# stevenmiller888/mlx-audio

Measured on AMD Instinct MI355X. Metric: audio-sec/sec (xRT), Kokoro-82M batch=32 fixed 128-phoneme utterances per GPU, higher is better.
Workload: dtype bf16; 1 GPU; Kokoro-82M bf16, batch=32/GPU fixed 128-phoneme utterances (T=130, F=650, 390000 samples = 16.25 s each), utterance-sharded over 1 GPU(s); global_batch=32, parallelism=utterance-shard x1, 2 batches in flight per GPU

## Files before the change

mlx-audio_amd/csrc/kk_conv_mfma4.hip:

```cpp
#include <stdlib.h>

#include "kk_common.h"
#include "kk_kernels.h"
#include "kk_conv_mfma_shared.h"

#define TR_NOW() 0ull
#define TR_ADD(slot, v) do { } while (0)
namespace {
typedef __bf16 bf16x2 __attribute__((ext_vector_type(2)));

typedef __bf16 bf16x8 __attribute__((ext_vector_type(8)));
typedef float f32x4 __attribute__((ext_vector_type(4)));

constexpr int BN = 128, CK = 64;
constexpr int XLD = 80;
constexpr int MAX_HALO = 50;
constexpr int CLD = BN;

constexpr int PS_BYTES = 2 * 3 * CK * 4;

template <int BM>
struct Geo {
  static constexpr int XROWS = BM + MAX_HALO;
  static constexpr int XS_BYTES = XROWS * XLD * 2;
  static constexpr int MAIN_BYTES = XS_BYTES + PS_BYTES;
  static constexpr int RPP = BM / 2;
  static constexpr int EPI_BYTES = RPP * CLD * 4;
  static constexpr int LDS_BYTES = MAIN_BYTES > EPI_BYTES ? MAIN_BYTES : EPI_BYTES;
  static constexpr int XREG = (XROWS * 8 + 255) / 256;
};


union U16 {
  uint4 u;
  bf16_t h[8];
};
union U32x8 {
  uint4 u[2];
  float f[8];
};

template <typename TO, int WM, int NRM>
__global__ __launch_bounds__(256, 2) __attribute__((amdgpu_waves_per_eu(2, 2))) void conv_mfma4_kernel(KKMfmaArgs a) {
  constexpr int BM = 2 * WM, MI16 = WM / 16;
  constexpr bool ACC16 = true;
  using G = Geo<BM>;
  constexpr int XREG = G::XREG;
  extern __shared__ __attribute__((aligned(16))) unsigned char smem[];
  bf16_t* Xs = (bf16_t*)smem;
  float* Ps = (float*)(smem + G::XS_BYTES);
  float* Cs = (float*)smem;

  const int tid = threadIdx.x, lane = tid & 63, wave = tid >> 6;
  const int wr = wave >> 1, wc = wave & 1;
  const int nphase = a.mode == KK_CONVT ? a.stride : 1;
  int bx, by, bz;
  {
    const int gx = gridDim.x, gy = gridDim.y, total = gx * gy * gridDim.z;
    int lid = blockIdx.x + gx * (blockIdx.y + gy * blockIdx.z);
    const int per = total / 8, rem = total - per * 8;
    const int xcd = lid & 7, idx = lid >> 3;
    lid = xcd * per + (xcd < rem ? xcd : rem) + idx;
    by = lid % gy;
    const int t = lid / gy;
    bx = t % gx;
    bz = t / gx;
  }
  const int b = bz / nphase, phase = bz - b * nphase;
  const int q0 = bx * BM, n0 = by * BN;
  const int Lin = kk_len(a.lin, b), Lout = kk_len(a.lout, b);

  int ntaps, off0, dstep, widx0, wstep;
  if (a.mode == KK_CONV) {
    ntaps = a.Kw; off0 = -a.pad; dstep = a.dil; widx0 = 0; wstep = 1;
  } else {
    const int k0 = (phase + a.pad) % a.stride;
    ntaps = (a.Kw - k0 + a.stride - 1) / a.stride;
    off0 = (phase + a.pad - k0) / a.stride; dstep = -1; widx0 = k0; wstep = a.stride;
  }
  const int min_off = dstep >= 0 ? off0 : off0 + (ntaps - 1) * dstep;
  const int halo = (ntaps - 1) * (dstep >= 0 ? dstep : -dstep);
  const int xrows = BM + halo;

  const int op_first = a.mode == KK_CONV ? q0 : phase + a.stride * q0;
  const bool tile_live = op_first < Lout;

  const unsigned long long tr0 = TR_NOW();
  unsigned long long tr_sx = 0, tr_sw = 0;
  (void)tr0; (void)tr_sx; (void)tr_sw;
  f32x4 acc[MI16][4];
#pragma unroll
  for (int i = 0; i < MI16; ++i)
#pragma unroll
    for (int j = 0; j < 4; ++j) acc[i][j] = f32x4{0.f, 0.f, 0.f, 0.f};

  if (tile_live) {
    const bf16_t* xb = a.x + (long long)b * a.xbs;
    const int nchunk = a.CinP / CK;
    const int nit = nchunk * ntaps;
    const int lin_hi = Lin > 0 ? Lin - 1 : 0;
    const int cin_real = a.Cin > 0 ? a.Cin : a.CinP;

#define KK_STG(name) name
#define KK_STG_XS Xs
#include "kk_conv_mfma_stage.h"
    uint4 q00, q01, q02, q03, q10, q11, q12, q13;
    const int nb = by;
    auto frag_ptr = [&](int it) __attribute__((always_inline)) -> const uint4* {
      const int chunk = it / ntaps, tap = it - chunk * ntaps;
      const long long blk = ((long long)(widx0 + tap * wstep) * (a.CoutP / BN) + nb) * nchunk + chunk;
      return (const uint4*)a.wf + blk * 1024 + (wc * 2) * 4 * 64 + lane;
    };
    load_x(0);
    {
      const uint4* fp = frag_ptr(0);
      q00 = fp[0 * 64]; q01 = fp[1 * 64]; q02 = fp[2 * 64]; q03 = fp[3 * 64];
      q10 = fp[4 * 64]; q11 = fp[5 * 64]; q12 = fp[6 * 64]; q13 = fp[7 * 64];
      asm volatile("" ::: "memory");
    }
    store_p(0);
    __syncthreads();
    store_x(0);
    __syncthreads();

    const int arow = wr * WM + (lane & 15);
    const int kofs = 8 * (lane >> 4);

    for (int it = 0; it < nit; ++it) {
      const int chunk = it / ntaps, tap = it - chunk * ntaps;
      const bool last_tap = tap == ntaps - 1;
      if (tap == 0 && chunk + 1 < nchunk) load_x(chunk + 1);
      const uint4* fn = frag_ptr(it + 1 < nit ? it + 1 : it);

      const int shift = (off0 + tap * dstep) - min_off;
      const bf16_t* xa = Xs + (arow + shift) * XLD + kofs;
      KK_MFMA_ITER(q00, q01, q02, q03, q10, q11, q12, q13)
      asm volatile("" ::: "memory");
      if (it + 1 < nit) {
        if (tap == 0 && chunk + 1 < nchunk) store_p(chunk + 1);
        if (last_tap) {
          __syncthreads();
          store_x(chunk + 1);
          __syncthreads();
        }
      }
    }
    __syncthreads();
  }

#include "kk_conv_mfma_epilogue.h"
}

template <int XR>
struct GeoWK {
  static constexpr int SROWS = XR == 7 ? 224 : 192 + MAX_HALO;
  static constexpr int SLAB = SROWS * XLD;
  static constexpr int XS_BYTES = 2 * SLAB * 2;
  static constexpr int MAIN_BYTES = XS_BYTES + PS_BYTES;
  static constexpr int RPP = 96;
  static constexpr int EPI_BYTES = RPP * CLD * 4;
  static constexpr int LDS_BYTES = MAIN_BYTES > EPI_BYTES ? MAIN_BYTES : EPI_BYTES;
};

template <int NRM, int XR>
__global__ __launch_bounds__(256, 2) __attribute__((amdgpu_waves_per_eu(2, 2))) void conv_mfma4_wholek_kernel(KKMfmaArgs a) {
  using TO = bf16_t;
  constexpr int WM = 96, BM = 2 * WM, MI16 = WM / 16, XREG = XR;
  constexpr bool ACC16 = true;
  using G = GeoWK<XR>;
  extern __shared__ __attribute__((aligned(16))) unsigned char smem[];
  bf16_t* Xs = (bf16_t*)smem;
  float* Ps = (float*)(smem + G::XS_BYTES);
  float* Cs = (float*)smem;

  const int tid = threadIdx.x, lane = tid & 63, wave = tid >> 6;
  const int wr = wave >> 1, wc = wave & 1;
  constexpr int nphase = 1, phase = 0;
  int bx, by, b;
  {
    const int gx = gridDim.x, gy = gridDim.y, total = gx * gy * gridDim.z;
    int lid = blockIdx.x + gx * (blockIdx.y + gy * blockIdx.z);
    const int per = total / 8, rem = total - per * 8;
    const int xcd = lid & 7, idx = lid >> 3;
    lid = xcd * per + (xcd < rem ? xcd : rem) + idx;
    by = lid % gy;
    const int t = lid / gy;
    bx = t % gx;
    b = t / gx;
  }
  const int q0 = bx * BM, n0 = by * BN;
  const int Lin = kk_len(a.lin, b), Lout = kk_len(a.lout, b);
  const int ntaps = a.Kw, off0 = -a.pad, dstep = a.dil, min_off = off0;
  const int xrows = BM + (ntaps - 1) * dstep;
  const bool tile_live = q0 < Lout;

  const unsigned long long tr0 = TR_NOW();
  (void)tr0;
  f32x4 acc[MI16][4];
#pragma unroll
  for (int i = 0; i < MI16; ++i)
#pragma unroll
    for (int j = 0; j < 4; ++j) acc[i][j] = f32x4{0.f, 0.f, 0.f, 0.f};

  if (tile_live) {
    const bf16_t* xb = a.x + (long long)b * a.xbs;
    const int nit = 2 * ntaps;
    const int lin_hi = Lin > 0 ? Lin - 1 : 0;
    const int cin_real = a.Cin > 0 ? a.Cin : a.CinP;

#define KK_STG(name) name##_s0
#define KK_STG_XS Xs
#include "kk_conv_mfma_stage.h"
#define KK_STG(name) name##_s1
#define KK_STG_XS (Xs + G::SLAB)
#include "kk_conv_mfma_stage.h"
    uint4 q00, q01, q02, q03, q10, q11, q12, q13;
    auto frag_ptr = [&](int it) __attribute__((always_inline)) -> const uint4* {
      const int chunk = it >= ntaps ? 1 : 0, tap = it - chunk * ntaps;
      const long long blk = ((long long)tap * (a.CoutP / BN) + by) * 2 + chunk;
      return (const uint4*)a.wf + blk * 1024 + (wc * 2) * 4 * 64 + lane;
    };
    load_x_s0(0);
    load_x_s1(1);
    {
      const uint4* fp = frag_ptr(0);
      q00 = fp[0 * 64]; q01 = fp[1 * 64]; q02 = fp[2 * 64]; q03 = fp[3 * 64];
      q10 = fp[4 * 64]; q11 = fp[5 * 64]; q12 = fp[6 * 64]; q13 = fp[7 * 64];
      asm volatile("" ::: "memory");
    }
    store_p_s0(0);
    store_p_s1(1);
    __syncthreads();
    store_x_s0(0);
    store_x_s1(1);
    __syncthreads();

    const int arow = wr * WM + (lane & 15);
    const int kofs = 8 * (lane >> 4);
    for (int it = 0; it + 1 < nit; ++it) {
      const int chunk = it >= ntaps ? 1 : 0, tap = it - chunk * ntaps;
      const uint4* fn = frag_ptr(it + 1);
      const bf16_t* xa = Xs + chunk * G::SLAB + (arow + tap * dstep) * XLD + kofs;
      KK_MFMA_ITER(q00, q01, q02, q03, q10, q11, q12, q13)
      asm volatile("" ::: "memory");
    }
    {
      const bf16_t* xa = Xs + G::SLAB + (arow + (ntaps - 1) * dstep) * XLD + kofs;
      KK_MFMA_ITER_LAST(q00, q01, q02, q03, q10, q11, q12, q13)
      asm volatile("" ::: "memory");
    }
    __syncthreads();
  }

#include "kk_conv_mfma_epilogue.h"
}

template <int NRM, int XR>
int launch_wholek(const KKMfmaArgs& a, int B, hipStream_t st) {
  using G = GeoWK<XR>;
  static KKDevOnce attr_once;
  if (attr_once.first()) {
    (void)hipFuncSetAttribute((const void*)conv_mfma4_wholek_kernel<NRM, XR>, hipFuncAttributeMaxDynamicSharedMemorySize, G::LDS_BYTES);
    attr_once.done();
  }
  dim3 grid(kk_cdiv(a.Q, 192), a.CoutP / BN, B);
  hipLaunchKernelGGL((conv_mfma4_wholek_kernel<NRM, XR>), grid, dim3(256), G::LDS_BYTES, st, a);
  KK_CHECK_LAUNCH();
  return 0;
}

template <typename TO, int WM, int NRM>
int launch_one(const KKMfmaArgs& a, int B, hipStream_t st) {
  using G = Geo<2 * WM>;
  static KKDevOnce attr_once;
  if (attr_once.first()) {
    (void)hipFuncSetAttribute((const void*)conv_mfma4_kernel<TO, WM, NRM>, hipFuncAttributeMaxDynamicSharedMemorySize, G::LDS_BYTES);
    attr_once.done();
  }
  const int nphase = a.mode == KK_CONVT ? a.stride : 1;
  dim3 grid(kk_cdiv(a.Q, 2 * WM), a.CoutP / BN, B * nphase);
  hipLaunchKernelGGL((conv_mfma4_kernel<TO, WM, NRM>), grid, dim3(256), G::LDS_BYTES, st, a);
  KK_CHECK_LAUNCH();
  return 0;
}

__global__ __launch_bounds__(256) void pack_w_frag_kernel(const bf16_t* w, bf16_t* wf, int Kw, int CoutP, int CinP) {
  const long long n = (long long)Kw * CoutP * CinP;
  for (long long e = (long long)blockIdx.x * 256 + threadIdx.x; e < n; e += (long long)gridDim.x * 256) {
    const int k = (int)(e % CinP);
    const long long r = e / CinP;
    const int cout = (int)(r % CoutP), tap = (int)(r / CoutP);
    wf[KK_MFMA4_PACK_INDEX(tap, cout, k, CoutP, CinP)] = w[e];
  }
}
}

int kk_launch_pack_w_frag(const void* w, void* wf, int Kw, int CoutP, int CinP, hipStream_t st) {
  if (CinP % CK != 0 || CoutP % BN != 0) return kk_fail("pack_w_frag: CinP must be a multiple of 64 and CoutP of 128");
  hipLaunchKernelGGL(pack_w_frag_kernel, dim3(1024), dim3(256), 0, st, (const bf16_t*)w, (bf16_t*)wf, Kw, CoutP, CinP);
  KK_CHECK_LAUNCH();
  return 0;
}

bool kk_mfma4_wholek_eligible(const KKMfmaArgs& a) {
  return a.mode == KK_CONV && a.stride == 1 && a.CinP == 2 * CK && a.dil >= 1 && (a.Kw - 1) * a.dil <= MAX_HALO;
}

int kk_launch_conv_mfma4(const KKMfmaArgs& a, int B, int out_dtype, hipStream_t st) {
  if (a.Q <= 0 || B <= 0) return 0;
  if (!a.wf) return kk_fail("conv_mfma4: fragment-order weights missing");
  const int nrm = a.nrm_a == nullptr ? 0 : (a.nrm_act == KK_ACT_SNAKE ? 1 : 2);
  if (nrm == 1 && a.nrm_C % 4 != 0) return kk_fail("conv_mfma: the fused Snake input needs a channel count that is a multiple of 4");
  KKMfmaArgs g = a;
  if (nrm == 2 && a.nrm_act != KK_ACT_LRELU) g.nrm_slope = 1.0f;
  if (out_dtype != KK_BF16) return kk_fail("conv_mfma4: bf16 output only");
  if (kk_mfma4_wholek_eligible(g) && !g.slabwise) {
    const bool x7 = (g.Kw - 1) * g.dil <= 32;
    if (nrm == 1) return x7 ? launch_wholek<1, 7>(g, B, st) : launch_wholek<1, 8>(g, B, st);
    if (nrm == 2) return x7 ? launch_wholek<2, 7>(g, B, st) : launch_wholek<2, 8>(g, B, st);
    return x7 ? launch_wholek<0, 7>(g, B, st) : launch_wholek<0, 8>(g, B, st);
  }
  if (nrm == 1) return launch_one<bf16_t, 96, 1>(g, B, st);
  if (nrm == 2) return launch_one<bf16_t, 96, 2>(g, B, st);
  return launch_one<bf16_t, 96, 0>(g, B, st);
}
```

mlx-audio_amd/csrc/kk_model.hip:

```cpp
#include <math.h>
#include <stdio.h>
#include <string.h>

#include <algorithm>
#include <functional>
#include <map>
#include <string>
#include <vector>

#include "../../include/kokoro_hip.h"
#include "kk_common.h"
#include "kk_kernels.h"
#include "kk_host.h"

static thread_local std::string g_err;
static const void* g_op_wfrag = nullptr;
static float g_op_post_slope = 0.f;
static int g_op_variant = 4;

int kk_fail(const char* msg) {
  g_err = msg ? msg : "unknown error";
  return -1;
}
extern "C" const char* kk_last_error(void) { return g_err.c_str(); }
// ... 527 lines not shown
  m->emb_ln_w = P.a.vec("bert.embeddings.LayerNorm.weight", E);
  m->emb_ln_b = P.a.vec("bert.embeddings.LayerNorm.bias", E);
  m->map_in = P.linear("bert.encoder.embedding_hidden_mapping_in", hs, E, true);
  const std::string lp = "bert.encoder.albert_layer_groups.0.albert_layers.0.";
  {
    std::vector<float> w((size_t)3 * hs * hs), b((size_t)3 * hs);
    const char* nm[3] = {"query", "key", "value"};
    for (int i = 0; i < 3; ++i) {
      std::vector<float> wi, bi;
      if (P.read(lp + "attention." + nm[i] + ".weight", (size_t)hs * hs, wi) && P.read(lp + "attention." + nm[i] + ".bias", hs, bi)) {
        memcpy(&w[(size_t)i * hs * hs], wi.data(), wi.size() * 4);
        memcpy(&b[(size_t)i * hs], bi.data(), bi.size() * 4);
      }
    }
    m->qkv = P.pack_oki(w, 3 * hs, 1, hs, &b);
    P.pack_fp8(m->qkv, w, 3 * hs, hs);
  }
  m->att_dense = P.linear(lp + "attention.dense", hs, hs, true);
  m->att_ln_w = P.a.vec(lp + "attention.LayerNorm.weight", hs);
  m->att_ln_b = P.a.vec(lp + "attention.LayerNorm.bias", hs);
  m->full_ln_w = P.a.vec(lp + "full_layer_layer_norm.weight", hs);
  m->full_ln_b = P.a.vec(lp + "full_layer_layer_norm.bias", hs);
  m->ffn = P.linear(lp + "ffn", c.plbert_intermediate, hs, true);
  m->ffn_out = P.linear(lp + "ffn_output", hs, c.plbert_intermediate, true);
  m->bert_encoder = P.linear("bert_encoder", H, hs, true);
  for (int i = 0; i < c.n_layer; ++i) {
    m->dur_lstms.push_back(P.lstm("predictor.text_encoder.lstms." + std::to_string(2 * i), H + S, H / 2));
    m->dur_adaln.push_back(SP.add("predictor.text_encoder.lstms." + std::to_string(2 * i + 1), H));
  }
  m->pred_lstm = P.lstm("predictor.lstm", H + S, H / 2);
  m->shared_lstm = P.lstm("predictor.shared", H + S, H / 2);
  {
    std::vector<float> wd, wt((size_t)c.max_dur * H);
    if (P.read("predictor.duration_proj.linear_layer.weight", (size_t)c.max_dur * H, wd)) {
      for (int o = 0; o < c.max_dur; ++o)
        for (int i = 0; i < H; ++i) wt[(size_t)i * c.max_dur + o] = wd[(size_t)o * H + i];
      m->dur_W = P.put(wt);
    }
  }
  m->dur_b = P.a.vec("predictor.duration_proj.linear_layer.bias", c.max_dur);
  for (int which = 0; which < 2; ++which) {
    const std::string nm = which == 0 ? "predictor.F0" : "predictor.N";
    ResBlk1d* blk = which == 0 ? m->f0blk : m->nblk;
    blk[0] = build_resblk1d(P, SP, nm + ".0", H, H, false);
    blk[1] = build_resblk1d(P, SP, nm + ".1", H, H / 2, true);
    blk[2] = build_resblk1d(P, SP, nm + ".2", H / 2, H / 2, false);
    (which == 0 ? m->f0_proj : m->n_proj) = P.conv_plain(nm + "_proj", 1, 1, H / 2);
  }
  m->te_emb = P.a.vec("text_encoder.embedding.weight", (size_t)c.n_token * H);
  for (int i = 0; i < c.n_layer; ++i) {
    const std::string is = std::to_string(i);
    m->te_cnn.push_back(P.convw("text_encoder.cnn." + is + ".0", H, c.text_encoder_kernel_size, H, true));
    m->te_ln_w.push_back(P.a.vec("text_encoder.cnn." + is + ".1.weight", H));
    m->te_ln_b.push_back(P.a.vec("text_encoder.cnn." + is + ".1.bias", H));
  }
  m->text_lstm = P.lstm("text_encoder.lstm", H, H / 2);
  m->enc = build_resblk1d(P, SD, "decoder.encode", H + 2, DH, false);
  for (int i = 0; i < 3; ++i) m->dec[i] = build_resblk1d(P, SD, "decoder.decode." + std::to_string(i), DH + 2 + 64, DH, false);
  m->dec[3] = build_resblk1d(P, SD, "decoder.decode.3", DH + 2 + 64, H, true);
  m->f0_conv = P.convw("decoder.F0_conv", 1, 3, 1, true);
  m->n_conv = P.convw("decoder.N_conv", 1, 3, 1, true);
  m->asr_res = P.convw("decoder.asr_res.0", 64, 1, H, true);
  const std::string g = "decoder.generator.";
  {
    std::vector<float> lw, lb;
    if (P.read(g + "m_source.l_linear.weight", 9, lw) && P.read(g + "m_source.l_linear.bias", 1, lb)) {
      m->lin_w = P.put(lw);
      m->lin_b = lb[0];
    }
  }
  const int C0 = c.upsample_initial_channel, nk = c.n_resblock_kernels;
  const int d135[3] = {1, 3, 5};
  for (int i = 0; i < c.n_upsamples; ++i) {
    const int cin = C0 >> i, cout = C0 >> (i + 1);
    const std::string is = std::to_string(i);
    m->ups[i] = P.convw_t(g + "ups." + is, cin, c.upsample_kernel_sizes[i], cout);
    if (i + 1 < c.n_upsamples) {
      int sf0 = 1;
      for (int j = i + 1; j < c.n_upsamples; ++j) sf0 *= c.upsample_rates[j];
      m->noise_conv[i] = P.conv_plain(g + "noise_convs." + is, cout, sf0 * 2, c.gen_istft_n_fft + 2);
      m->noise_conv_rows[i] = P.strided_rows(g + "noise_convs." + is, cout, sf0 * 2, c.gen_istft_n_fft + 2, sf0, (sf0 + 1) / 2, 64, &m->noise_rows_pad[i]);
      m->noise_res[i] = build_resblock1(P, SD, g + "noise_res." + is, cout, 7, d135);
    } else {
      m->noise_conv[i] = P.conv_plain(g + "noise_convs." + is, cout, 1, c.gen_istft_n_fft + 2);
      m->noise_res[i] = build_resblock1(P, SD, g + "noise_res." + is, cout, 11, d135);
    }
    for (int j = 0; j < nk; ++j)
      m->resblocks.push_back(
          build_resblock1(P, SD, g + "resblocks." + std::to_string(i * nk + j), cout, c.resblock_kernel_sizes[j], c.resblock_dilations[j]));
  }
  m->conv_post = P.convw(g + "conv_post", c.gen_istft_n_fft + 2, 7, C0 >> c.n_upsamples, true);
  if (P.ok() && m->adt == KK_BF16 && m->conv_post.mfma &&
      kk_head_eligible(m->conv_post.Cin, m->conv_post.Cout, m->conv_post.Kw, c.gen_istft_n_fft, c.gen_istft_hop_size)) {
    const ConvW& cp = m->conv_post;
    m->head_wf_off = P.a.alloc((kk_head_pack_elems() + 1) / 2);
    const uint16_t* src = (const uint16_t*)&P.a.pack[cp.wb_off];
    uint16_t* dst = (uint16_t*)&P.a.pack[m->head_wf_off];
    for (int t = 0; t < cp.Kw; ++t)
      for (int o = 0; o < cp.Cout; ++o)
        for (int i = 0; i < cp.Cin; ++i) dst[kk_head_pack_index(t, o, i)] = src[((size_t)t * cp.CoutP + o) * cp.CinP + i];
  }
  if (P.ok()) {
    SP.build(P, m->sp_wT, m->sp_b, m->Np);
    SD.build(P, m->sd_wT, m->sd_b, m->Nd);
  }
  if (!P.ok()) return kk_failf("kk_finalize: %s", P.a.err.c_str());

  KK_TRY(m->arena.upload((hipStream_t)stream, "kk_finalize"));
  ArenaVec* vecs[] = {&m->emb_word, &m->emb_pos, &m->emb_type, &m->emb_ln_w, &m->emb_ln_b, &m->att_ln_w, &m->att_ln_b, &m->full_ln_w,
                  &m->full_ln_b, &m->dur_W, &m->dur_b, &m->te_emb, &m->lin_w, &m->sp_wT, &m->sp_b, &m->sd_wT, &m->sd_b};
  for (ArenaVec* v : vecs) resolve(m, *v);
  ConvW* convs[] = {&m->map_in, &m->qkv, &m->att_dense, &m->ffn, &m->ffn_out, &m->bert_encoder, &m->f0_proj, &m->n_proj,
                    &m->f0_conv, &m->n_conv, &m->asr_res, &m->conv_post};
  for (ConvW* cw : convs) resolve(m, *cw);
  m->head_wf = m->head_wf_off ? (const bf16_t*)(m->arena.dev + m->head_wf_off) : nullptr;
  for (auto& l : m->dur_lstms) resolve(m, l);
  resolve(m, m->pred_lstm); resolve(m, m->shared_lstm); resolve(m, m->text_lstm);
  for (int i = 0; i < 3; ++i) { resolve(m, m->f0blk[i]); resolve(m, m->nblk[i]); }
  for (auto& cw : m->te_cnn) resolve(m, cw);
  for (auto& v : m->te_ln_w) resolve(m, v);
  for (auto& v : m->te_ln_b) resolve(m, v);
  resolve(m, m->enc);
  for (int i = 0; i < 4; ++i) resolve(m, m->dec[i]);
  for (int i = 0; i < c.n_upsamples; ++i) { resolve(m, m->noise_conv[i]); resolve(m, m->noise_conv_rows[i]); resolve(m, m->ups[i]); resolve(m, m->noise_res[i]); }
  for (auto& r : m->resblocks) resolve(m, r);
  m->finalized = true;
  return 0;
}

namespace {

struct Buf {
  void* p = nullptr;
  int ld = 0;
  long long bs = 0;
  int rows = 0;
  int dtype = KK_F32;
  Buf slice(int coff) const {
    Buf r = *this;
    r.p = p ? (char*)p + (size_t)coff * (dtype == KK_F32 ? 4 : 2) : nullptr;
    return r;
  }
  Buf row_offset(int r0) const {
    Buf r = *this;
    r.p = p ? (char*)p + (size_t)r0 * ld * (dtype == KK_F32 ? 4 : 2) : nullptr;
    r.rows = rows - r0;
    return r;
  }
};

struct ConvOpt {
  int mode = KK_CONV, stride = 1, pad = 0, dil = 1, in_shift = 0;
  float in_slope = 1.f;
  int act = KK_ACT_NONE;
  float act_slope = 0.f;
  float scale = 1.f;
  int accumulate = 0;
  const Buf* res = nullptr;
  const float* nrm_a = nullptr;
  const float* nrm_b = nullptr;
  int nrm_act = KK_ACT_NONE;
  float nrm_slope = 0.f;
  const float* nrm_alpha = nullptr;
  int nrm_C = 0;
  bool want_stats = false;
  bool pad_out_ok = false;
  double alg_taps_cin = 0;
  float post_slope = 1.f;
};

struct Ctx : Workspace {
  kk_model* m;
  kk_context* cx = nullptr;
  hipStream_t st;
  hipStream_t main_st = nullptr;
  bool side_on() const { return !dry && !cx->no_side && cx->side_stream && st != nullptr; }
  int fork_point(int k) {
    if (!side_on()) return 0;
    return hipEventRecord(cx->side_fork[k], st) == hipSuccess ? 0 : kk_fail("kk_forward: hipEventRecord failed");
  }
  int begin_side(int k) {
    if (!side_on()) return 0;
    if (hipStreamWaitEvent(cx->side_stream, cx->side_fork[k], 0) != hipSuccess) return kk_fail("kk_forward: hipStreamWaitEvent failed");
    main_st = st;
    st = cx->side_stream;
    return 0;
  }
  int end_side(int k) {
    if (!side_on() || !main_st) return 0;
    const hipError_t e = hipEventRecord(cx->side_join[k], st);
    st = main_st;
    main_st = nullptr;
    return e == hipSuccess ? 0 : kk_fail("kk_forward: hipEventRecord failed");
  }
  int join_side(int k) {
    if (!side_on()) return 0;
    return hipStreamWaitEvent(st, cx->side_join[k], 0) == hipSuccess ? 0 : kk_fail("kk_forward: hipStreamWaitEvent failed");
  }
  int B;
  int adt;

  Buf act(int rows, int ld, int dtype = -1) {
    Buf b;
    b.dtype = dtype < 0 ? adt : dtype;
    b.ld = ld;
    b.rows = rows;
    b.bs = (long long)rows * ld;
    b.p = raw((size_t)B * rows * ld * (b.dtype == KK_F32 ? 4 : 2));
    return b;
  }
  float* f32(size_t n) { return (float*)raw(n * 4); }
  int* i32(size_t n) { return (int*)raw(n * 4); }

  void prof_start() {
    if (dry || !cx->prof_on) return;
    const size_t i = cx->prof_rec.size();
    if (2 * i + 1 >= cx->prof_ev.size()) return;
    (void)hipEventRecord(cx->prof_ev[2 * i], st);
  }
  void prof_stop(int cls, double flops, double bytes) {
    if (dry || !cx->prof_on) return;
    const size_t i = cx->prof_rec.size();
    if (2 * i + 1 >= cx->prof_ev.size()) return;
    (void)hipEventRecord(cx->prof_ev[2 * i + 1], st);
    cx->prof_rec.push_back({cls, flops, bytes});
  }
  static double esz(int dt) { return dt == KK_F32 ? 4.0 : 2.0; }

  int dbg(const char* name, const Buf& b, int C) {
    if (dry) return 0;
    auto it = cx->dbg_over.find(name);
    if (it != cx->dbg_over.end())
      KK_TRY(kk_launch_convert(it->second, KK_F32, (long long)b.rows * C, C, b.p, b.dtype, b.bs, b.ld, C, b.rows, B, st));
    cx->dbg.map[name] = DebugNote{b.p, b.ld, b.bs, b.rows, C, b.dtype, B};
    return 0;
  }

  int conv(const ConvW& w, const Buf& x, KKLen lin, const Buf& out, KKLen lout, int Q, const ConvOpt& o) {
    if (dry) return 0;
    KKConvArgs a;
    memset(&a, 0, sizeof a);
    a.x = x.p; a.xbs = x.bs; a.ldx = x.ld;
    a.w = w.w; a.ldw = w.ldw; a.bias = w.b;
    a.out = out.p; a.obs = out.bs; a.ldo = out.ld;
    if (o.res) { a.res = o.res->p; a.rbs = o.res->bs; a.ldr = o.res->ld; }
    a.Cin = w.Cin; a.Cout = w.Cout; a.Kw = w.Kw;
    a.mode = o.mode; a.stride = o.stride; a.pad = o.pad; a.dil = o.dil; a.in_shift = o.in_shift;
    a.Q = Q; a.Lo_rows = out.rows;
    a.lin = lin; a.lout = lout;
    a.in_slope = o.in_slope; a.scale = o.scale; a.accumulate = o.accumulate; a.act = o.act; a.act_slope = o.act_slope;
    const double rows_out = o.mode == KK_CONVT ? (double)Q * o.stride : (double)Q;
    const double taps = o.mode == KK_CONVT ? (double)w.Kw / o.stride : (double)w.Kw;
    const double flops = 2.0 * B * rows_out * w.Cout * (o.alg_taps_cin > 0 ? o.alg_taps_cin : w.Cin * taps);
    const double bytes = B * (rows_out * w.Cout * esz(out.dtype) * (o.res ? 2.0 : 1.0) + (double)Q * (o.mode == KK_CONVT ? 1 : o.stride) * w.Cin * esz(x.dtype)) +
                         (double)w.Kw * w.Cin * w.Cout * 4.0;
    if (can_fp8(w, x, lin, out, lout, Q, o)) {
      KKFp8Args f;
      memset(&f, 0, sizeof f);
      f.aq = (const uint4*)q8_aq; f.as = (const unsigned char*)q8_as; f.wq = w.q8; f.ws = w.s8;
      f.M = B * x.rows; f.N = w.Cout; f.K = w.Cin; f.bias = w.b; f.out = (bf16_t*)out.p; f.ldo = out.ld; f.rows_per_item = x.rows;
      f.lout = lout; f.act = o.act;
      prof_start();
      int rc = kk_launch_mxfp8_quant_rows(x.p, x.ld, f.M, f.K, q8_aq, q8_as, st);
      if (rc == 0) rc = kk_launch_linear_mxfp8(f, st);
      prof_stop(10, flops, B * (double)Q * (w.Cin * 2.0 + w.Cin * 1.03 * 2.0 + w.Cout * 2.0) + (double)w.Cin * w.Cout * 1.03);
      return rc;
    }
    const bool lr_size_ok = cx->linrows_mode == 1 || (cx->linrows_mode == 0 && (long long)B * Q <= 1024);
    if (lr_size_ok && w.wl && w.Kw == 1 && can_mfma(w, x, out, o) && out.dtype == KK_BF16 && o.mode == KK_CONV && o.stride == 1 && o.pad == 0 && o.dil == 1 &&
        o.in_shift == 0 && !o.nrm_a && !o.want_stats && !o.res && !o.accumulate && o.in_slope == 1.f && o.scale == 1.f && o.post_slope == 1.f &&
        (o.act == KK_ACT_NONE || o.act == KK_ACT_GELU) && Q == x.rows && Q == out.rows && lin.len == lout.len && lin.mul == lout.mul && lin.add == lout.add &&
        !cx->no_v4) {
      KKLinMfmaArgs f;
      memset(&f, 0, sizeof f);
      f.x = (const bf16_t*)x.p; f.xbs = x.bs; f.ldx = x.ld; f.wl = w.wl; f.bias = w.b; f.Nb = w.CoutP;
      f.out = (bf16_t*)out.p; f.obs = out.bs; f.ldo = out.ld; f.K = w.Cin; f.N = w.Cout8; f.rows = Q; f.items = B;
      f.flat = (x.bs == (long long)x.rows * x.ld && out.bs == (long long)out.rows * out.ld) ? 1 : 0;
      f.len = lout; f.act = o.act;
      prof_start();
      const int rc = kk_launch_linear_rows_mfma(f, st);
      prof_stop(1, flops, bytes);
      return rc;
    }
    if (can_mfma(w, x, out, o)) {
      KKMfmaArgs g;
      memset(&g, 0, sizeof g);
      g.nrm_a = o.nrm_a; g.nrm_b = o.nrm_b; g.nrm_stride = fz_stride; g.nrm_act = o.nrm_act; g.nrm_slope = o.nrm_slope;
      g.nrm_alpha = o.nrm_alpha; g.nrm_C = o.nrm_C;
      g.x = (const bf16_t*)x.p; g.xbs = x.bs; g.ldx = x.ld; g.w = w.wb; g.CinP = w.CinP; g.Cin = w.Cin; g.CoutP = w.CoutP; g.bias = w.b;
      g.out = out.p; g.obs = out.bs; g.ldo = out.ld;
      if (o.res) { g.res = o.res->p; g.rbs = o.res->bs; g.ldr = o.res->ld; }
      g.Cout = w.Cout8; g.Kw = w.Kw; g.mode = o.mode; g.stride = o.stride; g.pad = o.pad; g.dil = o.dil; g.in_shift = o.in_shift;
      g.Q = Q; g.Lo_rows = out.rows; g.lin = lin; g.lout = lout; g.in_slope = o.in_slope; g.scale = o.scale; g.accumulate = o.accumulate;
      g.act = o.act; g.act_slope = o.act_slope; g.post_slope = o.post_slope;
      if (o.want_stats) {
        last_ntiles = kk_cdiv(Q, KK_MFMA_TILE_ROWS) * (o.mode == KK_CONVT ? o.stride : 1);
        if ((size_t)B * last_ntiles * 2 * w.Cout > fz_part_floats) return kk_fail("internal: statistics scratch too small");
        g.stat_part = fz_part;
        g.stat_ntiles = last_ntiles;
      }
      const bool v4 = w.wf && out.dtype == KK_BF16 && !cx->no_v4;
      g.wf = v4 ? w.wf : nullptr;
      const bool v5 = v4 && cx->v5_mode != 2 && (cx->v5_mode == 1 || g.Kw >= 9 || (g.Kw >= 7 && g.CinP >= 256)) && B <= 256 && kk_mfma5_eligible(g, out.dtype);
      g.slabwise = (cx->no_wholek || !g.nrm_a) ? 1 : 0;
      int Bl = B;
      if (!v5 && B > 1 && w.Kw == 1 && o.mode == KK_CONV && o.stride == 1 && o.pad == 0 && o.dil == 1 && o.in_shift == 0 && !o.nrm_a && !o.want_stats &&
          Q == x.rows && Q == out.rows && Q % 192 != 0 && x.bs == (long long)x.rows * x.ld && out.bs == (long long)out.rows * out.ld &&
          (!o.res || (o.res->rows == out.rows && o.res->bs == (long long)o.res->rows * o.res->ld)) && (long long)B * Q < (1ll << 30)) {
        g.flat_T = Q;
        g.flat_len = lout;
        g.Q = B * Q;
        g.Lo_rows = B * out.rows;
        g.lin = KKLen{nullptr, 0, B * Q};
        g.lout = KKLen{nullptr, 0, B * Q};
        Bl = 1;
      }
      prof_start();
      const int rc = v5 ? kk_launch_conv_mfma5(g, Bl, out.dtype, st) : v4 ? kk_launch_conv_mfma4(g, Bl, out.dtype, st) : kk_launch_conv_mfma(g, Bl, out.dtype, st);
      prof_stop(1, flops, bytes);
      return rc;
    }
    if (o.nrm_a || o.want_stats) return kk_fail("internal: fused norm requested on a conv that is not MFMA eligible");
    prof_start();
    const int rc = kk_launch_conv_generic(a, B, x.dtype, out.dtype, st);
    prof_stop(0, flops, bytes);
    return rc;
  }

  void* q8_aq = nullptr;
  void* q8_as = nullptr;
  size_t q8_rows = 0, q8_K = 0;
  bool can_fp8(const ConvW& w, const Buf& x, KKLen lin, const Buf& out, KKLen lout, int Q, const ConvOpt& o) const {
    return w.fp8 && !cx->no_fp8 && !cx->force_generic && q8_aq && x.dtype == KK_BF16 && out.dtype == KK_BF16 && w.Kw == 1 && o.mode == KK_CONV &&
           o.stride == 1 && o.pad == 0 && o.dil == 1 && o.in_shift == 0 && o.in_slope == 1.f && !o.res && o.scale == 1.f && !o.accumulate &&
           (o.act == KK_ACT_NONE || o.act == KK_ACT_GELU) && !o.nrm_a && !o.want_stats && x.rows == out.rows && Q == x.rows &&
           x.bs == (long long)x.rows * x.ld && out.bs == (long long)out.rows * out.ld && x.ld % 8 == 0 && !((uintptr_t)x.p & 15) &&
           lin.len == lout.len && lin.mul == lout.mul && lin.add == lout.add && (size_t)B * x.rows <= q8_rows && (size_t)w.Cin <= q8_K;
  }

  bool can_mfma(const ConvW& w, const Buf& x, const Buf& out, const ConvOpt& o) const {
    const bool al16 = !(((uintptr_t)x.p | (uintptr_t)out.p | (uintptr_t)(o.res ? o.res->p : nullptr)) & 15);
    const bool cout_ok = w.Cout == w.Cout8 || (out.ld >= w.Cout8 && !o.res && !o.accumulate && o.pad_out_ok);
    return w.mfma && cout_ok && x.dtype == KK_BF16 && (out.dtype == KK_BF16 || out.dtype == KK_F32) && (!o.res || o.res->dtype == out.dtype) &&
           kk_mfma_eligible(w.Cin, w.Cout8, w.Kw, o.mode, o.stride, o.dil) && x.ld >= w.CinP && x.ld % 8 == 0 && out.ld % 8 == 0 &&
           (!o.res || o.res->ld % 8 == 0) && al16 && !cx->force_generic;
  }

  float* fz_part = nullptr;
  size_t fz_part_floats = 0;
  float* fz_pa[2] = {nullptr, nullptr};
  float* fz_pb[2] = {nullptr, nullptr};
  int fz_stride = 0;
  int fz_flip = 0;
  int last_ntiles = 0;
  int finalize(int C, KKLen len, const float* gb, int gbs, float* mean, float* rstd, float** pa, float** pb) {
    if (dry) return 0;
    KKStatsArgs a;
    memset(&a, 0, sizeof a);
    a.C = C; a.len = len; a.partial = fz_part; a.nchunk = last_ntiles; a.mean = mean; a.rstd = rstd; a.eps = 1e-5f; a.fused = 1;
    if (gb) {
      fz_flip ^= 1;
      a.gb = gb; a.gbs = gbs; a.pa = fz_pa[fz_flip]; a.pb = fz_pb[fz_flip]; a.pstride = fz_stride; a.Cp = rup(C, 64);
      *pa = a.pa; *pb = a.pb;
    }
    return kk_launch_norm_finalize(a, B, st);
  }
  int fold(int C, KKLen len, const float* mean, const float* rstd, const float* gb, int gbs, float** pa, float** pb) {
    if (dry) return 0;
    KKStatsArgs a;
    memset(&a, 0, sizeof a);
    fz_flip ^= 1;
    a.C = C; a.len = len; a.mean = const_cast<float*>(mean); a.rstd = const_cast<float*>(rstd); a.fused = 2; a.gb = gb; a.gbs = gbs;
    a.pa = fz_pa[fz_flip]; a.pb = fz_pb[fz_flip]; a.pstride = fz_stride; a.Cp = rup(C, 64);
    *pa = a.pa; *pb = a.pb;
    return kk_launch_norm_finalize(a, B, st);
  }

  float* st_partial = nullptr;
  float* st_mean = nullptr;
  float* st_rstd = nullptr;
  static int rows_per_chunk(int rows_per_frame) { return rows_per_frame >= 20 ? 512 : 64; }
  int Fcap = 0;

  int stats(const Buf& x, int C, int Lmax, KKLen len) {
    if (dry) return 0;
    KKStatsArgs a;
    memset(&a, 0, sizeof a);
    a.x = x.p; a.xbs = x.bs; a.ldx = x.ld; a.C = C; a.Lmax = Lmax; a.len = len;
    a.partial = st_partial; a.rows_per_chunk = rows_per_chunk(Fcap > 0 ? Lmax / Fcap : 1); a.mean = st_mean; a.rstd = st_rstd; a.eps = 1e-5f;
    prof_start();
    const int rc = kk_launch_instnorm_stats(a, B, x.dtype, st);
    prof_stop(2, 3.0 * B * Lmax * C, (double)B * Lmax * C * esz(x.dtype));
    return rc;
  }
  int adain(const Buf& x, int C, KKLen len_in, const Buf& out, int Cpad, int Lmax_out, const float* gb, int gbs, int act, float slope,
            const float* alpha, int pool, const float* pool_w, const float* pool_b) {
    if (dry) return 0;
    KKAdainArgs a;
    memset(&a, 0, sizeof a);
    a.x = x.p; a.xbs = x.bs; a.ldx = x.ld; a.out = out.p; a.obs = out.bs; a.ldo = out.ld;
    a.C = C; a.Cpad = Cpad; a.Lmax_out = Lmax_out; a.len_in = len_in;
    a.mean = st_mean; a.rstd = st_rstd; a.gb = gb; a.gbs = gbs; a.act = act; a.slope = slope; a.alpha = alpha;
    a.pool = pool; a.pool_w = pool_w; a.pool_b = pool_b; a.fast = adt == KK_BF16;
    prof_start();
    const int rc = kk_launch_adain_act(a, B, x.dtype, st);
    prof_stop(3, 8.0 * B * Lmax_out * C, (double)B * Lmax_out * C * esz(x.dtype) * (pool ? 1.5 : 2.0));
    return rc;
  }
  int layernorm(const Buf& x, const Buf* res, const Buf& out, int C, int Lmax, KKLen len, const float* w, const float* b, const float* gb,
                int gbs, float eps, int act, float slope) {
    if (dry) return 0;
    KKLnArgs a;
    memset(&a, 0, sizeof a);
    a.x = x.p; a.xbs = x.bs; a.ldx = x.ld;
    if (res) { a.res = res->p; a.rbs = res->bs; a.ldr = res->ld; }
    a.out = out.p; a.obs = out.bs; a.ldo = out.ld; a.C = C; a.Lmax = Lmax; a.len = len; a.w = w; a.bias = b; a.gb = gb; a.gbs = gbs;
    a.eps = eps; a.act = act; a.slope = slope;
    prof_start();
    const int rc = kk_launch_layernorm(a, B, x.dtype, st);
    prof_stop(6, 8.0 * B * Lmax * C, (double)B * Lmax * C * esz(x.dtype) * (res ? 3.0 : 2.0));
    return rc;
  }
  int lstm(const LstmW& l, const Buf& x, int Cin_ld_unused, float* xproj, const Buf& out, int Lmax, KKLen len) {
    (void)Cin_ld_unused;
    if (dry) return 0;
    Buf xp;
    xp.p = xproj; xp.ld = 8 * l.H; xp.bs = (long long)Lmax * 8 * l.H; xp.rows = Lmax; xp.dtype = KK_F32;
    ConvOpt o;
    KK_TRY(conv(l.in, x, len, xp, len, Lmax, o));
    KKLstmArgs a;
    memset(&a, 0, sizeof a);
    a.xproj = xproj; a.whT = l.whT.p; a.out = out.p; a.obs = out.bs; a.ldo = out.ld; a.H = l.H; a.Lmax = Lmax; a.len = len;
    prof_start();
    const int rc = (l.whb && adt == KK_BF16 && !cx->force_generic) ? kk_launch_lstm_h256_bf16(a, l.whb, B, out.dtype, st)
                                                                    : kk_launch_lstm(a, B, out.dtype, st);
    prof_stop(4, 2.0 * B * Lmax * 2 * 4 * l.H * l.H, 2.0 * Lmax * 4 * l.H * l.H * 4.0 * B);
    return rc;
  }
};


int run_resblk1d(Ctx& c, const ResBlk1d& r, const Buf& x, KKLen lin, int Lmax_in, const Buf& out, const float* style, int gbs,
                 Buf& bufA, Buf& bufB, Buf& bufC) {
  const int Lmax_out = r.up ? 2 * Lmax_in : Lmax_in;
  KKLen lout = lin;
  if (r.up) { lout.mul = lin.mul * 2; lout.add = lin.add * 2; }
  {
    ConvOpt p1, p2;
    p1.pad = p2.pad = 1;
    p2.res = r.learned ? &out : &x;
    const Buf& c1in = r.up ? bufA : x;
    if (c.adt == KK_BF16 && c.fz_part && !c.cx->no_fusion && c.can_mfma(r.conv1, c1in, bufB, p1) && c.can_mfma(r.conv2, bufB, out, p2) &&
        (!r.learned || c.can_mfma(r.sc, x, out, ConvOpt()))) {
      float *pa = nullptr, *pb = nullptr;
      KK_TRY(c.stats(x, r.Cin, Lmax_in, lin));
      ConvOpt o1;
      o1.pad = 1;
      o1.want_stats = true;
      if (r.up) {
        KK_TRY(c.adain(x, r.Cin, lin, bufA, rup(r.Cin, 64) <= bufA.ld ? rup(r.Cin, 64) : r.Cin, Lmax_out, style + r.n1.off, gbs,
                       KK_ACT_LRELU, 0.2f, nullptr, 1, r.pool_w.p, r.pool_b.p));
      } else {
        KK_TRY(c.fold(r.Cin, lin, c.st_mean, c.st_rstd, style + r.n1.off, gbs, &pa, &pb));
        o1.nrm_a = pa; o1.nrm_b = pb; o1.nrm_act = KK_ACT_LRELU; o1.nrm_slope = 0.2f; o1.nrm_C = r.Cin;
      }
      KK_TRY(c.conv(r.conv1, c1in, lout, bufB, lout, Lmax_out, o1));
      KK_TRY(c.finalize(r.Cout, lout, style + r.n2.off, gbs, nullptr, nullptr, &pa, &pb));
      ConvOpt o2;
      o2.pad = 1;
      o2.scale = 0.70710678118654752440f;
      o2.nrm_a = pa; o2.nrm_b = pb; o2.nrm_act = KK_ACT_LRELU; o2.nrm_slope = 0.2f; o2.nrm_C = r.Cout;
      if (r.learned) {
        ConvOpt os;
        os.in_shift = r.up ? 1 : 0;
        KK_TRY(c.conv(r.sc, x, lin, out, lout, Lmax_out, os));
        o2.res = &out;
      } else {
        o2.res = &x;
      }
      return c.conv(r.conv2, bufB, lout, out, lout, Lmax_out, o2);
    }
  }
  KK_TRY(c.stats(x, r.Cin, Lmax_in, lin));
  KK_TRY(c.adain(x, r.Cin, lin, bufA, rup(r.Cin, 64) <= bufA.ld ? rup(r.Cin, 64) : r.Cin, Lmax_out, style + r.n1.off, gbs, KK_ACT_LRELU,
                 0.2f, nullptr, r.up ? 1 : 0, r.pool_w.p, r.pool_b.p));
  ConvOpt o1;
  o1.pad = 1;
  KK_TRY(c.conv(r.conv1, bufA, lout, bufB, lout, Lmax_out, o1));
  KK_TRY(c.stats(bufB, r.Cout, Lmax_out, lout));
  KK_TRY(c.adain(bufB, r.Cout, lout, bufC, r.Cout, Lmax_out, style + r.n2.off, gbs, KK_ACT_LRELU, 0.2f, nullptr, 0, nullptr, nullptr));
  ConvOpt o2;
  o2.pad = 1;
  o2.scale = 0.70710678118654752440f;
  if (r.learned) {
    ConvOpt os;
    os.in_shift = r.up ? 1 : 0;
    KK_TRY(c.conv(r.sc, x, lin, out, lout, Lmax_out, os));
    o2.res = &out;
  } else {
    o2.res = &x;
  }
  KK_TRY(c.conv(r.conv2, bufC, lout, out, lout, Lmax_out, o2));
  return 0;
}

int run_resblock1(Ctx& c, const ResBlock1& r, const Buf& x_in, const Buf& y, Buf& t1, Buf& t2, int Lmax, KKLen len, const float* style,
                  int gbs, const Buf* acc, float acc_scale, int acc_accumulate, bool x_stats_ready = false, float post_slope = 1.f) {
  {
    ConvOpt p1, p2;
    p1.dil = r.dil[2]; p1.pad = (r.k * r.dil[2] - r.dil[2]) / 2;
    p2.pad = (r.k - 1) / 2; p2.res = &x_in;
    if (c.adt == KK_BF16 && c.fz_part && !c.cx->no_fusion && c.can_mfma(r.c1[0], x_in, t2, p1) && c.can_mfma(r.c2[0], t2, y, p2) &&
        (!acc || c.can_mfma(r.c2[2], t2, *acc, p2))) {
      float *pa = nullptr, *pb = nullptr;
      if (!x_stats_ready) KK_TRY(c.stats(x_in, r.C, Lmax, len));
      KK_TRY(c.fold(r.C, len, c.st_mean, c.st_rstd, style + r.a1[0].off, gbs, &pa, &pb));
      for (int j = 0; j < 3; ++j) {
        const Buf& src = j == 0 ? x_in : y;
        ConvOpt o1;
        o1.dil = r.dil[j];
        o1.pad = (r.k * r.dil[j] - r.dil[j]) / 2;
        o1.nrm_a = pa; o1.nrm_b = pb; o1.nrm_act = KK_ACT_SNAKE; o1.nrm_alpha = r.al1[j].p; o1.nrm_C = r.C;
        o1.want_stats = true;
        KK_TRY(c.conv(r.c1[j], src, len, t2, len, Lmax, o1));
        KK_TRY(c.finalize(r.C, len, style + r.a2[j].off, gbs, nullptr, nullptr, &pa, &pb));
        ConvOpt o2;
        o2.pad = (r.k - 1) / 2;
        o2.res = &src;
        o2.nrm_a = pa; o2.nrm_b = pb; o2.nrm_act = KK_ACT_SNAKE; o2.nrm_alpha = r.al2[j].p; o2.nrm_C = r.C;
        if (j == 2 && acc) {
          o2.scale = acc_scale;
          o2.accumulate = acc_accumulate;
          o2.post_slope = post_slope;
          KK_TRY(c.conv(r.c2[j], t2, len, *acc, len, Lmax, o2));
        } else {
          o2.want_stats = j < 2;
          KK_TRY(c.conv(r.c2[j], t2, len, y, len, Lmax, o2));
          if (j < 2) KK_TRY(c.finalize(r.C, len, style + r.a1[j + 1].off, gbs, nullptr, nullptr, &pa, &pb));
        }
      }
      return 0;
    }
  }
  for (int j = 0; j < 3; ++j) {
    const Buf& src = j == 0 ? x_in : y;
    KK_TRY(c.stats(src, r.C, Lmax, len));
    KK_TRY(c.adain(src, r.C, len, t1, r.C, Lmax, style + r.a1[j].off, gbs, KK_ACT_SNAKE, 0.f, r.al1[j].p, 0, nullptr, nullptr));
    ConvOpt o1;
    o1.dil = r.dil[j];
    o1.pad = (r.k * r.dil[j] - r.dil[j]) / 2;
    KK_TRY(c.conv(r.c1[j], t1, len, t2, len, Lmax, o1));
    KK_TRY(c.stats(t2, r.C, Lmax, len));
    KK_TRY(c.adain(t2, r.C, len, t1, r.C, Lmax, style + r.a2[j].off, gbs, KK_ACT_SNAKE, 0.f, r.al2[j].p, 0, nullptr, nullptr));
    ConvOpt o2;
    o2.pad = (r.k - 1) / 2;
    o2.res = &src;
    if (j == 2 && acc) {
      o2.scale = acc_scale;
      o2.accumulate = acc_accumulate;
      KK_TRY(c.conv(r.c2[j], t1, len, *acc, len, Lmax, o2));
    } else {
      KK_TRY(c.conv(r.c2[j], t1, len, y, len, Lmax, o2));
    }
  }
  return 0;
}

struct TextState {
  Buf d, t_en;
  int* pred_dur = nullptr;
};

int run_text(Ctx& c, int Tmax, const int* ids, const int* lens, const float* ref_s, const float* speed, TextState& ts, int* pred_dur_out) {
  kk_model* m = c.m;
  kk_context* cx = c.cx;
  (void)cx;
  const kk_config& cf = m->cfg;
  const int H = cf.hidden_dim, hs = cf.plbert_hidden, E = cf.plbert_embedding, B = c.B;
  const KKLen lT{lens, 1, 0};
  if (m->q_group && m->adt == KK_BF16) {
    c.q8_rows = (size_t)B * Tmax;
    c.q8_K = (size_t)std::max(std::max(hs, E), (int)cf.plbert_intermediate);
    c.q8_aq = c.raw(kk_mxfp8_q_bytes((int)c.q8_rows, (int)c.q8_K));
    c.q8_as = c.raw(kk_mxfp8_s_bytes((int)c.q8_rows, (int)c.q8_K));
    if (c.dry) c.q8_aq = nullptr;
  }
  KK_TRY(c.fork_point(0));
  Buf e = c.act(Tmax, E), x = c.act(Tmax, hs), qkv = c.act(Tmax, 3 * hs), ctxb = c.act(Tmax, hs), att = c.act(Tmax, hs),
      ff = c.act(Tmax, cf.plbert_intermediate), tmp = c.act(Tmax, hs);
  if (!c.dry) {
    KKEmbedArgs ea;
    memset(&ea, 0, sizeof ea);
    ea.ids = ids; ea.word = m->emb_word.p; ea.pos = m->emb_pos.p; ea.type = m->emb_type.p; ea.ln_w = m->emb_ln_w.p; ea.ln_b = m->emb_ln_b.p;
    ea.out = e.p; ea.obs = e.bs; ea.ldo = e.ld; ea.E = E; ea.Tmax = Tmax; ea.len = lT; ea.eps = 1e-12f;
    KK_TRY(kk_launch_albert_embed(ea, B, e.dtype, c.st));
  }
  ConvOpt plain;
  KK_TRY(c.conv(m->map_in, e, lT, x, lT, Tmax, plain));
  for (int layer = 0; layer < cf.plbert_layers; ++layer) {
    KK_TRY(c.conv(m->qkv, x, lT, qkv, lT, Tmax, plain));
    if (!c.dry) {
      KKAttnArgs aa;
      memset(&aa, 0, sizeof aa);
      aa.qkv = qkv.p; aa.bs = qkv.bs; aa.ld = qkv.ld; aa.out = ctxb.p; aa.obs = ctxb.bs; aa.ldo = ctxb.ld;
      aa.heads = cf.plbert_heads; aa.hs = hs; aa.Tmax = Tmax; aa.len = lT; aa.scale = 0.125f;
      c.prof_start();
      KK_TRY(kk_launch_attention(aa, B, qkv.dtype, c.st));
// ... 689 lines not shown
```

Measured before the change: 15380 audio-sec/sec.

## Add double-buffered ring conv kernel for multi-chunk MFMA4 convolutions

Adds a new MFMA4 convolution kernel that double-buffers input-channel chunks in LDS. It loads the next chunk's input and weight fragments while the current chunk's taps are computed, with one barrier per chunk. It also remaps block IDs to spread them across the XCDs. It is routed to convs with CinP>=192 and either Kw=1 without fused norm or Kw 3/7 with fused Snake. The slabwise gating changes so that unnormalised wide convs can reach it. The new path carries more register and LDS pressure and adds code complexity.

```diff
diff --git a/mlx-audio_amd/csrc/kk_conv_mfma4.hip b/mlx-audio_amd/csrc/kk_conv_mfma4.hip
--- a/mlx-audio_amd/csrc/kk_conv_mfma4.hip
+++ b/mlx-audio_amd/csrc/kk_conv_mfma4.hip
@@ -256,6 +256,153 @@
 }
 
 template <int NRM, int XR>
+__global__ __launch_bounds__(256, 2) __attribute__((amdgpu_waves_per_eu(2, 2))) void conv_mfma4_ring_kernel(KKMfmaArgs a) {
+  using TO = bf16_t;
+  constexpr int WM = 96, BM = 2 * WM, MI16 = WM / 16, XREG = XR;
+  constexpr bool ACC16 = true;
+  using G = GeoWK<7>;
+  extern __shared__ __attribute__((aligned(16))) unsigned char smem[];
+  bf16_t* Xs = (bf16_t*)smem;
+  float* Ps = (float*)(smem + G::XS_BYTES);
+  float* Cs = (float*)smem;
+
+  const int tid = threadIdx.x, lane = tid & 63, wave = tid >> 6;
+  const int wr = wave >> 1, wc = wave & 1;
+  constexpr bool K1 = XR == 6;
+  static_assert(!(K1 && NRM), "the one-tap schedule carries no parameter pipeline");
+  constexpr int nphase = 1, phase = 0;
+  int bx, by, b;
+  {
+    const int gx = gridDim.x, gy = gridDim.y, total = gx * gy * gridDim.z;
+    int lid = blockIdx.x + gx * (blockIdx.y + gy * blockIdx.z);
+    const int per = total / 8, rem = total - per * 8;
+    const int xcd = lid & 7, idx = lid >> 3;
+    lid = xcd * per + (xcd < rem ? xcd : rem) + idx;
+    by = lid % gy;
+    const int t = lid / gy;
+    bx = t % gx;
+    b = t / gx;
+  }
+  const int q0 = bx * BM, n0 = by * BN;
+  const int Lin = kk_len(a.lin, b), Lout = kk_len(a.lout, b);
+  const int ntaps = K1 ? 1 : a.Kw, off0 = -a.pad, dstep = K1 ? 1 : a.dil, min_off = off0;
+  const int xrows = BM + (ntaps - 1) * dstep;
+  const bool tile_live = q0 < Lout;
+
+  const unsigned long long tr0 = TR_NOW();
+  (void)tr0;
+  f32x4 acc[MI16][4];
+#pragma unroll
+  for (int i = 0; i < MI16; ++i)
+#pragma unroll
+    for (int j = 0; j < 4; ++j) acc[i][j] = f32x4{0.f, 0.f, 0.f, 0.f};
+
+  if (tile_live) {
+    const bf16_t* xb = a.x + (long long)b * a.xbs;
+    const int nchunk = a.CinP / CK;
+    const int lin_hi = Lin > 0 ? Lin - 1 : 0;
+    const int cin_real = a.Cin > 0 ? a.Cin : a.CinP;
+
+    int stbuf = 0;
+#define KK_STG(name) name
+#define KK_STG_XS (Xs + stbuf)
+#include "kk_conv_mfma_stage.h"
+    auto load_p = [&](int chunk) __attribute__((always_inline)) -> float4 {
+      if (!NRM) return make_float4(0.f, 0.f, 0.f, 0.f);
+      const int which = __builtin_amdgcn_readfirstlane(tid >> 6), c = chunk * CK + (tid & 15) * 4;
+      const float* base = (NRM == 1 && which == 2) ? a.nrm_alpha : (which == 1 ? a.nrm_b : a.nrm_a) + (long long)b * a.nrm_stride;
+      const int off = (NRM == 1 && which == 2) ? (c + 3 < a.nrm_C ? c : 0) : c;
+      return *(const float4*)(base + off);
+    };
+    uint4 q00, q01, q02, q03, q10, q11, q12, q13;
+    auto frag_ptr = [&](int chunk, int tap) __attribute__((always_inline)) -> const uint4* {
+      const long long blk = ((long long)tap * (a.CoutP / BN) + by) * nchunk + chunk;
+      return (const uint4*)a.wf + blk * 1024 + (wc * 2) * 4 * 64 + lane;
+    };
+    const int arow = wr * WM + (lane & 15);
+    const int kofs = 8 * (lane >> 4);
+#define KK_RING_ITER(C, TAP, FC, FT)                                                                            \
+    {                                                                                                             \
+      const uint4* fn = frag_ptr(FC, FT);                                                                         \
+      const bf16_t* xa = Xs + ((C) & 1) * G::SLAB + (arow + (TAP) * dstep) * XLD + kofs;                       \
+      KK_MFMA_ITER(q00, q01, q02, q03, q10, q11, q12, q13)                                                       \
+      asm volatile("" ::: "memory");                                                                              \
+    }
+
+    load_x(0);
+    {
+      const uint4* fp = frag_ptr(0, 0);
+      q00 = fp[0 * 64]; q01 = fp[1 * 64]; q02 = fp[2 * 64]; q03 = fp[3 * 64];
+      q10 = fp[4 * 64]; q11 = fp[5 * 64]; q12 = fp[6 * 64]; q13 = fp[7 * 64];
+      asm volatile("" ::: "memory");
+    }
+    float4 pnext = load_p(1);
+    store_p(0);
+    if (NRM) {
+      preg = pnext;
+      store_p(1);
+    }
+    __syncthreads();
+    store_x(0);
+    __syncthreads();
+
+    int c = 0;
+    if (K1) {
+#pragma unroll 1
+      for (; c + 1 < nchunk; ++c) {
+        load_x(c + 1);
+        KK_RING_ITER(c, 0, c + 1, 0)
+        stbuf = ((c + 1) & 1) * G::SLAB;
+        store_x(c + 1);
+        __syncthreads();
+      }
+    } else {
+#pragma unroll 1
+      for (; c + 1 < nchunk; ++c) {
+        pnext = load_p(c + 2 < nchunk ? c + 2 : c + 1);
+        load_x(c + 1);
+        KK_RING_ITER(c, 0, c, 1)
+        for (int tap = 1; tap < ntaps; ++tap) {
+          const bool lt = tap + 1 == ntaps;
+          KK_RING_ITER(c, tap, lt ? c + 1 : c, lt ? 0 : tap + 1)
+        }
+        if (NRM && c + 2 < nchunk) {
+          preg = pnext;
+          store_p(c + 2);
+        }
+        stbuf = ((c + 1) & 1) * G::SLAB;
+        store_x(c + 1);
+        __syncthreads();
+      }
+    }
+    for (int tap = 0; tap + 1 < ntaps; ++tap) KK_RING_ITER(c, tap, c, tap + 1)
+    {
+      const bf16_t* xa = Xs + (c & 1) * G::SLAB + (arow + (ntaps - 1) * dstep) * XLD + kofs;
+      KK_MFMA_ITER_LAST(q00, q01, q02, q03, q10, q11, q12, q13)
+      asm volatile("" ::: "memory");
+    }
+#undef KK_RING_ITER
+    __syncthreads();
+  }
+
+#include "kk_conv_mfma_epilogue.h"
+}
+
+template <int NRM, int XR>
+int launch_ring(const KKMfmaArgs& a, int B, hipStream_t st) {
+  using G = GeoWK<7>;
+  static KKDevOnce attr_once;
+  if (attr_once.first()) {
+    (void)hipFuncSetAttribute((const void*)conv_mfma4_ring_kernel<NRM, XR>, hipFuncAttributeMaxDynamicSharedMemorySize, G::LDS_BYTES);
+    attr_once.done();
+  }
+  dim3 grid(kk_cdiv(a.Q, 192), a.CoutP / BN, B);
+  hipLaunchKernelGGL((conv_mfma4_ring_kernel<NRM, XR>), grid, dim3(256), G::LDS_BYTES, st, a);
+  KK_CHECK_LAUNCH();
+  return 0;
+}
+
+template <int NRM, int XR>
 int launch_wholek(const KKMfmaArgs& a, int B, hipStream_t st) {
   using G = GeoWK<XR>;
   static KKDevOnce attr_once;
@@ -304,6 +451,11 @@
 
 bool kk_mfma4_wholek_eligible(const KKMfmaArgs& a) {
   return a.mode == KK_CONV && a.stride == 1 && a.CinP == 2 * CK && a.dil >= 1 && (a.Kw - 1) * a.dil <= MAX_HALO;
+}
+
+static bool ring_eligible(const KKMfmaArgs& a, int nrm) {
+  if (a.mode != KK_CONV || a.stride != 1 || a.CinP < 3 * CK || a.dil < 1 || (a.Kw - 1) * a.dil > 32) return false;
+  return a.Kw == 1 ? nrm == 0 : (nrm == 1 && (a.Kw == 3 || a.Kw == 7));
 }
 
 int kk_launch_conv_mfma4(const KKMfmaArgs& a, int B, int out_dtype, hipStream_t st) {
@@ -320,6 +472,9 @@
     if (nrm == 2) return x7 ? launch_wholek<2, 7>(g, B, st) : launch_wholek<2, 8>(g, B, st);
     return x7 ? launch_wholek<0, 7>(g, B, st) : launch_wholek<0, 8>(g, B, st);
   }
+  if (!g.slabwise && ring_eligible(g, nrm)) {
+    return nrm == 1 ? launch_ring<1, 7>(g, B, st) : launch_ring<0, 6>(g, B, st);
+  }
   if (nrm == 1) return launch_one<bf16_t, 96, 1>(g, B, st);
   if (nrm == 2) return launch_one<bf16_t, 96, 2>(g, B, st);
   return launch_one<bf16_t, 96, 0>(g, B, st);
diff --git a/mlx-audio_amd/csrc/kk_model.hip b/mlx-audio_amd/csrc/kk_model.hip
--- a/mlx-audio_amd/csrc/kk_model.hip
+++ b/mlx-audio_amd/csrc/kk_model.hip
@@ -853,7 +853,7 @@
       const bool v4 = w.wf && out.dtype == KK_BF16 && !cx->no_v4;
       g.wf = v4 ? w.wf : nullptr;
       const bool v5 = v4 && cx->v5_mode != 2 && (cx->v5_mode == 1 || g.Kw >= 9 || (g.Kw >= 7 && g.CinP >= 256)) && B <= 256 && kk_mfma5_eligible(g, out.dtype);
-      g.slabwise = (cx->no_wholek || !g.nrm_a) ? 1 : 0;
+      g.slabwise = (cx->no_wholek || (!g.nrm_a && g.CinP < 192)) ? 1 : 0;
       int Bl = B;
       if (!v5 && B > 1 && w.Kw == 1 && o.mode == KK_CONV && o.stride == 1 && o.pad == 0 && o.dil == 1 && o.in_shift == 0 && !o.nrm_a && !o.want_stats &&
           Q == x.rows && Q == out.rows && Q % 192 != 0 && x.bs == (long long)x.rows * x.ld && out.bs == (long long)out.rows * out.ld &&
```

After: 15550 audio-sec/sec (median of 6 runs). 1.01x the previous value.
